# cindytsai/multigrid_poisson_solver

Hardware: AMD Instinct MI355X
Metric: vcycle_mlups (higher is better)
Workload: dtype f64; 1 GPU; V(3,3)-cycle N=8192^2 fp64, 11 levels to N=8, red-black GS(1e-7) coarse solve, cycle-file driver (eager, stream smoother: temporally blocked wave-streaming kernels on the large levels, register-tile kernels on the levels 65..1024, one-workgroup LDS kernel below; halos recomputed, neighbours via DPP lane shifts); N=8192, levels=11

## Files before the change

multigrid_poisson_solver_amd/csrc/mg_stream_impl.h:

```cpp
#include <hip/hip_runtime.h>

#include <type_traits>
#include <utility>

#include <algorithm>
#include <cstdlib>
#include <vector>

#include "mg_divconst.h"
#include "mg_internal.h"
#include "mg_lane_ops.h"

#if !defined(MG_REAL) || !defined(MG_REAL_NS)
#error "define MG_REAL (double|float) and MG_REAL_NS (f64|f32) before including mg_stream_impl.h"
#endif

namespace mg {
namespace k {
namespace MG_REAL_NS {

typedef MG_REAL real_t;

constexpr int PF_DEFAULT = 2;
#ifndef MG_WAVES_PER_WG
#define MG_WAVES_PER_WG 4
#endif
constexpr int WAVES_PER_WG = MG_WAVES_PER_WG;
constexpr int MAX_S = 4;
#ifndef MG_PF
#define MG_PF 2
#endif

constexpr bool recompute_instantiated(int pre, int steps)
{
    return MG_PF == 2 && pre >= 1 && steps >= 1 && pre <= MAX_S && steps <= MAX_S && pre + steps <= 6;
}

enum InMode { IN_LOAD = 0, IN_ZERO = 1, IN_PROLONG = 2 };

typedef real_t real2_t __attribute__((ext_vector_type(2)));
typedef real_t real4_t __attribute__((ext_vector_type(4)));

struct StreamParams {
    int N;
    real_t dx2, inv;
    const real_t *in;
    const real_t *F;
    real_t *out;
    real_t *D;
    int d_sign;
    double *part;
    long long *trace;
    int cols4;
    int rows_per_chunk;
    int groups;
    int n_blocks;
    int row_base, rows_local, own_y0, own_y1;
    int norm_y0, norm_y1;
    double *out_wide;
    int coarse_base, coarse_rows;
    int raw_norm;
    int nt_min_n;
    int no_out;
    int pre;
    int fc_base, fc_rows;
    const real_t *coarse;
    int Nc;
    const int *p_orow, *p_ocol;
    const real_t *p_rhi, *p_rlo, *p_chi, *p_clo;
    real_t c_dx, c_dx_rcp;
    real_t *Fc;
    int M;
    const int *r_inv;
    const real_t *r_w;
    const real_t *r_wf;
    const NodeBatchItem *batch;
    int part_stride;
    int n_batch;
    double *const *err_outs;
    real_t cw;
    int wt;
    real_t dc;
    int sh;
};


typedef const int __attribute__((address_space(4))) *const_int_ptr;
typedef const real_t __attribute__((address_space(4))) *const_real_ptr;
__device__ __forceinline__ int table_i(const int *t, int i) { return ((const_int_ptr)(uintptr_t)t)[i]; }
__device__ __forceinline__ real_t table_d(const real_t *t, int i) { return ((const_real_ptr)(uintptr_t)t)[i]; }

template <int COLS>
struct Row {
    real_t v[COLS];
};

#ifndef MG_ZERO_LEVEL1
#define MG_ZERO_LEVEL1 1
#endif
#ifndef MG_NT_LOADS
#define MG_NT_LOADS 0
#endif
template <int COLS, bool NT = false>
__device__ __forceinline__ Row<COLS> load_row(const real_t *__restrict__ row, unsigned col_bytes)
{
    Row<COLS> r;
    const char *a = reinterpret_cast<const char *>(row) + col_bytes;
    if constexpr (COLS == 2) {
        const real2_t t = NT ? __builtin_nontemporal_load(reinterpret_cast<const real2_t *>(a)) : *reinterpret_cast<const real2_t *>(a);
        r.v[0] = t.x;
        r.v[1] = t.y;
    } else if constexpr (COLS == 4) {
        const real4_t t = NT ? __builtin_nontemporal_load(reinterpret_cast<const real4_t *>(a)) : *reinterpret_cast<const real4_t *>(a);
        r.v[0] = t.x;
        r.v[1] = t.y;
        r.v[2] = t.z;
        r.v[3] = t.w;
    } else {
        r.v[0] = *reinterpret_cast<const real_t *>(a);
    }
    return r;
}

template <int COLS, bool NT>
__device__ __forceinline__ void store_row(real_t *__restrict__ row, unsigned col_bytes, const Row<COLS> &r)
{
    char *a = reinterpret_cast<char *>(row) + col_bytes;
    if constexpr (COLS == 2) {
        real2_t t;
        t.x = r.v[0];
        t.y = r.v[1];
        if constexpr (NT) __builtin_nontemporal_store(t, reinterpret_cast<real2_t *>(a));
        else *reinterpret_cast<real2_t *>(a) = t;
    } else if constexpr (COLS == 4) {
        real4_t t;
        t.x = r.v[0];
        t.y = r.v[1];
        t.z = r.v[2];
        t.w = r.v[3];
        if constexpr (NT) __builtin_nontemporal_store(t, reinterpret_cast<real4_t *>(a));
        else *reinterpret_cast<real4_t *>(a) = t;
    } else {
        *reinterpret_cast<real_t *>(a) = r.v[0];
    }
}

template <int S, bool RESTRICT, int COLS = 2>
struct Halo {
    static constexpr int A = COLS > 2 ? COLS : 2;
    static constexpr int value = (S + (RESTRICT ? 2 : 1) + A - 1) / A * A;
};


template <int NCV>
struct CoarseV {
    real_t v[NCV];
};
template <int NCV>
__device__ __forceinline__ CoarseV<NCV> load_coarse(const real_t *__restrict__ coarse, int Nc, int base, int rows, int row,
                                                    const unsigned (&col)[NCV])
{
    CoarseV<NCV> c;
    int r = row - base;
    r = r < 0 ? 0 : (r < rows - 1 ? r : rows - 1);
    const char *b = reinterpret_cast<const char *>(coarse + (size_t)r * Nc);
#pragma unroll
    for (int q = 0; q < NCV; ++q) c.v[q] = *reinterpret_cast<const real_t *>(b + col[q]);
    return c;
}


template <int NCV>
__device__ __forceinline__ CoarseV<NCV> load_coarse_local(const real_t *__restrict__ coarse, int Nc, int local_row, const unsigned (&col)[NCV])
{
    CoarseV<NCV> c;
    const char *b = reinterpret_cast<const char *>(coarse + (size_t)local_row * Nc);
#pragma unroll
    for (int q = 0; q < NCV; ++q) c.v[q] = *reinterpret_cast<const real_t *>(b + col[q]);
    return c;
}

template <class F, int... K>
__device__ __forceinline__ void unrolled_while(F &&f, std::integer_sequence<int, K...>)
{
    (void)(f(std::integral_constant<int, K>{}) && ...);
}

#ifndef MG_WPE_DOWN
#define MG_WPE_DOWN 0
#endif
template <int S, int COLS, int IN, bool RESTRICT, int PRE>
struct WavesPerSimd {
    static constexpr int min = (MG_WPE_DOWN > 0 && sizeof(real_t) == 8 && COLS == 2 && IN == 1  && RESTRICT && S <= 3) ? MG_WPE_DOWN : 1;
};

#ifndef MG_LDS_RING
#define MG_LDS_RING 1
#endif
#ifndef MG_PACKED_F32
#define MG_PACKED_F32 1
#endif
typedef float pk_t __attribute__((ext_vector_type(2)));
__device__ __forceinline__ pk_t pk(float a, float b)
{
    pk_t r;
    r.x = a;
    r.y = b;
    return r;
}
__device__ __forceinline__ pk_t pk_fma(pk_t a, pk_t b, pk_t c) { return __builtin_elementwise_fma(a, b, c); }
__device__ __forceinline__ pk_t pk_div_by_const(pk_t x, float c, float rc)
{
    const pk_t cc = pk(c, c), rr = pk(rc, rc);
    pk_t q = x * rr;
    pk_t r = pk_fma(-q, cc, x);
    q = pk_fma(r, rr, q);
    r = pk_fma(-q, cc, x);
    return pk_fma(r, rr, q);
}
template <int COLS, int PRE>
struct LdsRing {
    static constexpr bool value = MG_LDS_RING && PRE > 0 && (COLS == 2 || (COLS == 4 && sizeof(real_t) == 4));
};
template <int COLS> struct RingVec { typedef real_t full; typedef real_t half; };
template <> struct RingVec<2> { typedef real2_t full; typedef real_t half; };
template <> struct RingVec<4> { typedef real4_t full; typedef real2_t half; };
template <int COLS>
__device__ __forceinline__ typename RingVec<COLS>::full ring_pack(const Row<COLS> &r)
{
    typename RingVec<COLS>::full t;
    if constexpr (COLS == 1) t = r.v[0];
    else {
#pragma unroll
        for (int j = 0; j < COLS; ++j) t[j] = r.v[j];
    }
    return t;
}
template <int COLS>
__device__ __forceinline__ Row<COLS> ring_unpack(const typename RingVec<COLS>::full &t)
{
    Row<COLS> r;
    if constexpr (COLS == 1) r.v[0] = t;
    else {
#pragma unroll
        for (int j = 0; j < COLS; ++j) r.v[j] = t[j];
    }
    return r;
}
#ifndef MG_PF_UP
#define MG_PF_UP 3
#endif
#ifndef MG_PF_DOWN
#define MG_PF_DOWN 3
#endif
#ifndef MG_WPE_UP
#define MG_WPE_UP 2
#endif

template <bool SH>
__device__ __forceinline__ real_t minus_centre(real_t a, real_t u, real_t dc)
{
    if constexpr (SH) return a - dc * u;
    else return minus4(a, u);
}

template <int S, int COLS, int IN, bool RESTRICT, int PF = PF_DEFAULT, bool NT = false, int PRE = 0, bool WT = false, bool SH = false>
__global__ __launch_bounds__(64 * WAVES_PER_WG) __attribute__((amdgpu_waves_per_eu(LdsRing<COLS, PRE>::value ? MG_WPE_UP : WavesPerSimd<S, COLS, IN, RESTRICT, PRE>::min)))
void k_jacobi_stream(const StreamParams p)
{
    static_assert(COLS == 2 || COLS == 4 || (IN != IN_PROLONG && !RESTRICT), "fused transfer stages need column pairs");
    static_assert(COLS != 4 || sizeof(real_t) == 4, "4 columns per lane = one 16-byte access: fp32 fields only");
    constexpr int NCV = COLS / 2 + 2;
    constexpr int NS = COLS >= 2 ? COLS / 2 : 1;
    static_assert(PRE == 0 || (IN == IN_PROLONG && !RESTRICT), "recomputed pre-smoothing belongs to the fused `1` node");
    static_assert(!WT || (PRE == 0 && sizeof(real_t) == 8), "the weighted sweep: fp64 nodes that store and re-read U");
    static_assert(!SH || WT, "the screened operator is a form of the weighted sweep");
    constexpr int L = S + PRE;
    constexpr bool LDSR = LdsRing<COLS, PRE>::value;
    constexpr bool HALF = LDSR;
    constexpr bool PACKED = MG_PACKED_F32 && (COLS == 2 || COLS == 4) && sizeof(real_t) == 4;
#ifndef MG_TB_DIRECT
#define MG_TB_DIRECT 0
#endif
    constexpr bool TB_DIRECT = LDSR && MG_TB_DIRECT;
    constexpr int NB = LDSR ? 8 : (PF + L + 2 <= 8 ? 8 : 16);
    constexpr int NFR = LDSR ? (PF < 4 ? 4 : 8) : NB;
    static_assert((LDSR ? L + 2 <= NB : PF + L + 2 <= NB) && PF < 8, "the F ring has NB slots, the U ring 4 or 8");
    static_assert(!LDSR || (IN == IN_PROLONG && !RESTRICT), "the LDS ring belongs to the recomputing `1` node");
    typedef typename RingVec<COLS>::full ring_t;
    typedef typename RingVec<COLS>::half ringh_t;
    __shared__ ring_t s_g[LDSR ? WAVES_PER_WG : 1][LDSR ? NB : 1][LDSR ? 64 : 1];
    __shared__ ringh_t s_f[LDSR ? WAVES_PER_WG : 1][LDSR ? NB : 1][LDSR ? 64 : 1];
    constexpr int W = 64 * COLS;
    constexpr int H = Halo<L, RESTRICT, COLS>::value;
    constexpr int OW = W - 2 * H;

#ifdef MG_STREAM_TRACE
    const long long tr0 = wall_clock64();
#endif
    const int per_xcd = (p.n_blocks + 7) >> 3;
    const int tile = (int)(blockIdx.x & 7) * per_xcd + (int)(blockIdx.x >> 3);
    if (tile >= p.n_blocks) return;
    const real_t *a_in = p.in, *a_F = p.F, *a_coarse = p.coarse;
    real_t *a_out = p.out, *a_Fc = p.Fc;
    double *a_part = p.part;
    if (p.batch) {
        typedef const NodeBatchItem __attribute__((address_space(4))) *item_ptr;
        const item_ptr b = (item_ptr)(uintptr_t)(p.batch + blockIdx.y);
        a_in = static_cast<const real_t *>(b->in);
        a_F = static_cast<const real_t *>(b->F);
        a_coarse = static_cast<const real_t *>(b->coarse);
        a_out = static_cast<real_t *>(b->out);
        a_Fc = static_cast<real_t *>(b->Fc);
        if (a_part) a_part += (size_t)blockIdx.y * (size_t)p.part_stride;
    }
    const int chunk = tile / p.groups;
    const int group = tile - chunk * p.groups;

    const int lane = threadIdx.x & 63;
    const int wave = threadIdx.x >> 6;
    const int strip = group * WAVES_PER_WG + wave;
    const int N = p.N;
    const int own_x0 = strip * OW;
    if (own_x0 >= N) {
        if (a_part && lane == 0) a_part[(size_t)tile * WAVES_PER_WG + wave] = 0.0;
        return;
    }
    const int y0 = p.own_y0 + chunk * p.rows_per_chunk;
    int y1 = y0 + p.rows_per_chunk;
    if (y1 > p.own_y1) y1 = p.own_y1;
    if (y0 >= p.own_y1) return;
    const int av_lo = p.row_base > 0 ? p.row_base : 0;
    const int av_hi = p.row_base + p.rows_local < N ? p.row_base + p.rows_local : N;

    const int xl = own_x0 - H + lane * COLS;
    bool col_in[COLS], col_edge[COLS];
    bool lane_owns = true;
    real_t qc[COLS];
#pragma unroll
    for (int j = 0; j < COLS; ++j) {
        const int x = xl + j;
        col_in[j] = x >= 0 && x < N;
        col_edge[j] = x <= 0 || x >= N - 1;
        lane_owns = lane_owns && x >= own_x0 && x < own_x0 + OW && x < N;
        qc[j] = col_edge[j] ? real_t(0.0) : (WT ? p.cw : real_t(0.25));
    }
    int nm_even[COLS], nm_odd[COLS];
#pragma unroll
    for (int j = 0; j < COLS; ++j) {
        const bool mine = lane_owns && !col_edge[j];
        nm_even[j] = (mine && ((xl + j) & 1) == 0) ? -1 : 0;
        nm_odd[j] = (mine && ((xl + j) & 1) != 0) ? -1 : 0;
    }
    const bool lane_loads = col_in[0] && col_in[COLS - 1];
    const real_t dx2 = p.dx2, inv = p.inv;
    const real_t dc = SH ? p.dc : real_t(4.0);
    const bool want_res = RESTRICT || p.D != nullptr || p.part != nullptr;
    const unsigned col_off = (unsigned)(xl < 0 ? 0 : (xl > N - COLS ? N - COLS : xl)) * (unsigned)sizeof(real_t);
    const unsigned col_st = (unsigned)(xl < 0 ? 0 : xl) * (unsigned)sizeof(real_t);
    const unsigned row_bytes = (unsigned)N * (unsigned)sizeof(real_t);

    unsigned pc_col[NCV];
    int pc_cell[COLS];
    real_t pc_hi[COLS], pc_lo[COLS];
    real_t hA[COLS], hB[COLS];
#pragma unroll
    for (int q = 0; q < NCV; ++q) pc_col[q] = 0u;
#pragma unroll
    for (int j = 0; j < COLS; ++j) {
        pc_cell[j] = 0;
        pc_hi[j] = pc_lo[j] = hA[j] = hB[j] = real_t(0.0);
    }
    int c_row = -0x40000000;
    if constexpr (IN == IN_PROLONG) {
        if (lane_loads) {
            const int pc_base = p.p_ocol[xl];
            const int last = p.Nc - 1;
#pragma unroll
            for (int j = 0; j < COLS; ++j) {
                pc_cell[j] = p.p_ocol[xl + j] - pc_base;
                pc_hi[j] = p.p_chi[xl + j];
                pc_lo[j] = p.p_clo[xl + j];
            }
#pragma unroll
            for (int q = 0; q < NCV; ++q) pc_col[q] = (unsigned)(pc_base + q < last ? pc_base + q : last) * (unsigned)sizeof(real_t);
        }
    }
    auto interpolate = [&](const CoarseV<NCV> &c, real_t (&h)[COLS]) {
#pragma unroll
        for (int j = 0; j < COLS; ++j) {
            real_t ca = c.v[0], cb = c.v[1];
#pragma unroll
            for (int q = 1; q + 1 < NCV; ++q) {
                const bool here = pc_cell[j] == q;
                ca = here ? c.v[q] : ca;
                cb = here ? c.v[q + 1] : cb;
            }
            h[j] = ca * pc_hi[j] + cb * pc_lo[j];
        }
    };

    int rc_col[NS];
    bool rc_shift[NS];
    real_t rw_a[NS], rw_b[NS];
    Row<COLS> d_prev;
#pragma unroll
    for (int j = 0; j < COLS; ++j) d_prev.v[j] = 0.0;
#pragma unroll
    for (int q = 0; q < NS; ++q) {
        rc_col[q] = -1;
        rc_shift[q] = false;
        rw_a[q] = rw_b[q] = real_t(0.0);
    }
    if constexpr (RESTRICT) {
        if (lane_owns) {
#pragma unroll
            for (int q = 0; q < NS; ++q) {
                const int ca = p.r_inv[xl + 2 * q], cb = p.r_inv[xl + 2 * q + 1];
                rc_col[q] = ca >= 0 ? ca : cb;
                rc_shift[q] = ca < 0 && cb >= 0;
                if (rc_col[q] >= 0) {
                    rw_a[q] = p.r_w[rc_col[q]];
                    rw_b[q] = real_t(1.0) - rw_a[q];
                }
            }
        }
    }
    const bool first_col_lane = RESTRICT && lane_owns && xl == 0;
    const bool last_col_lane = RESTRICT && lane_owns && xl + COLS == N;
    if constexpr (RESTRICT) {
        for (int edge = 0; edge < 2; ++edge) {
            if (edge == 0 ? (y0 != 0) : (y1 != N)) continue;
            real_t *row = a_Fc + (size_t)((edge == 0 ? 0 : p.M - 1) - p.fc_base) * p.M;
#pragma unroll
            for (int q = 0; q < NS; ++q)
                if (rc_col[q] >= 0) row[rc_col[q]] = 0.0;
            if (first_col_lane) row[0] = 0.0;
            if (last_col_lane) row[p.M - 1] = 0.0;
        }
    }
    real_t ms[COLS];
#pragma unroll
    for (int j = 0; j < COLS; ++j) ms[j] = col_edge[j] ? real_t(0.0) : (p.d_sign < 0 ? real_t(-1.0) : real_t(1.0));

    constexpr bool EVEN_START = COLS >= 2;
    const int y0e = EVEN_START ? (y0 & ~1) : y0;
    const int y_first = y0e - (L + 1);
    const int T = (y1 - y0e) + 2 * (L + 1) + (RESTRICT ? 1 : 0);
    const int y_end = y_first + T;

    int tb_own = -1, tbn_own = -1;
    real_t tb_yh = 0.0, tb_yl = 0.0, tbn_yh = 0.0, tbn_yl = 0.0;
    int tb_rc = -1, tbn_rc = -1;
    real_t tb_rw = 0.0, tbn_rw = 0.0;
    auto load_own_block = [&](int first_row) {
        const int y = first_row + lane;
        const bool ok = y >= av_lo && y < av_hi && y < y_end;
        const int yc = y < 0 ? 0 : (y < N ? y : N - 1);
        const int v = p.p_orow[yc];
        tbn_own = ok ? v : -1;
    };
    auto load_weight_block = [&](int first_row) {
        const int y = first_row + lane;
        const int yc = y < 0 ? 0 : (y < N ? y : N - 1);
        tbn_yh = p.p_rhi[yc];
        tbn_yl = p.p_rlo[yc];
    };
    auto load_restrict_block = [&](int first_row) {
        const int y = first_row + lane;
        const bool ok = y >= y0 && y < y1;
        const int yc = y < 0 ? 0 : (y < N ? y : N - 1);
        const int v = p.r_inv[yc];
        const real_t w = p.r_wf[yc];
        tbn_rc = ok ? v : -1;
        tbn_rw = w;
    };
    const int yp_first = y_first - PRE;
    if constexpr (IN == IN_PROLONG) {
        load_own_block(yp_first);
        tb_own = tbn_own;
        load_weight_block(yp_first);
        tb_yh = tbn_yh;
        tb_yl = tbn_yl;
    }
    if constexpr (RESTRICT) {
        load_restrict_block(y_first - (L + 2));
        tb_rc = tbn_rc;
        tb_rw = tbn_rw;
    }

    Row<COLS> older[L + 1], newer[L + 1];
#pragma unroll
    for (int l = 0; l <= L; ++l)
#pragma unroll
        for (int j = 0; j < COLS; ++j) older[l].v[j] = newer[l].v[j] = 0.0;
    constexpr int NU = PF < 4 ? 4 : 8;
    Row<COLS> fr[NFR], pu[NU];
    CoarseV<NCV> pc[NU];
    int q_own[NU];
#pragma unroll
    for (int k = 0; k < NFR; ++k)
#pragma unroll
        for (int j = 0; j < COLS; ++j) fr[k].v[j] = 0.0;
#pragma unroll
    for (int k = 0; k < NU; ++k) {
#pragma unroll
        for (int j = 0; j < COLS; ++j) pu[k].v[j] = 0.0;
#pragma unroll
        for (int q = 0; q < NCV; ++q) pc[k].v[q] = 0.0;
        q_own[k] = -1;
    }

    if constexpr (LDSR) {
#pragma unroll
        for (int k = 0; k < NB; ++k) {
            s_g[wave][k][lane] = ring_t(real_t(0.0));
            s_f[wave][k][lane] = ringh_t(real_t(0.0));
        }
    }

    const char *in_b = reinterpret_cast<const char *>(a_in), *f_b = reinterpret_cast<const char *>(a_F);
    const int yc_first = y_first < av_lo ? av_lo : (y_first < av_hi ? y_first : av_hi - 1);
    unsigned long long ld_off = (unsigned long long)(yc_first - p.row_base) * row_bytes;
    int ld_t = 0;
    long long st_off = (long long)(y_first - L - p.row_base) * (long long)row_bytes;
    const unsigned inner_rows = (unsigned)(av_hi - av_lo - 1);

    auto fetch = [&](int u8) {
        if constexpr (IN != IN_ZERO && PRE == 0) pu[u8 % NU] = load_row<COLS, (MG_NT_LOADS >= 2)>(reinterpret_cast<const real_t *>(in_b + ld_off), col_off);
        fr[u8 % NFR] = load_row<COLS, (MG_NT_LOADS >= 1)>(reinterpret_cast<const real_t *>(f_b + ld_off), col_off);
        if constexpr (IN == IN_PROLONG) {
            const int own_s = lane_value(tb_own, ld_t & 63);
            q_own[u8 % NU] = own_s;
            const int cr = own_s + 1 - p.coarse_base;
            const int crc = cr < 0 ? 0 : (cr < p.coarse_rows - 1 ? cr : p.coarse_rows - 1);
            pc[u8 % NU] = load_coarse_local<NCV>(a_coarse, p.Nc, crc, pc_col);
        }
        ++ld_t;
        ld_off += ((unsigned)(y_first + ld_t - av_lo - 1) < inner_rows) ? row_bytes : 0u;
    };
#pragma unroll
    for (int k = 0; k < PF; ++k) fetch(k);

    if constexpr (IN == IN_PROLONG) {
        const int ys = yp_first > av_lo ? yp_first : av_lo;
        if (ys < av_hi && ys < y_end) {
            const int i0 = table_i(p.p_orow, ys);
            const CoarseV<NCV> c0 = load_coarse<NCV>(a_coarse, p.Nc, p.coarse_base, p.coarse_rows, i0, pc_col);
            interpolate(c0, hB);
            c_row = i0 - 1;
        }
    }

#ifdef MG_STREAM_TRACE
    const long long tr1 = wall_clock64();
#endif
    Row<COLS> gq[L + 1];
#pragma unroll
    for (int l = 0; l <= L; ++l)
#pragma unroll
        for (int j = 0; j < COLS; ++j) gq[l].v[j] = 0.0;
    double acc = 0.0;
    const unsigned rows_own = (unsigned)(y1 - y0), rows_norm = (unsigned)(p.norm_y1 - p.norm_y0);
    int nm_k0[COLS], nm_k1[COLS];
    const bool first_odd = ((y_first - L - 1) & 1) != 0;
    {
#pragma unroll
        for (int j = 0; j < COLS; ++j) {
            nm_k0[j] = first_odd ? nm_odd[j] : nm_even[j];
            nm_k1[j] = first_odd ? nm_even[j] : nm_odd[j];
        }
    }

    for (int t0 = 0; t0 < T; t0 += NB) {
        if ((t0 & 63) == 64 - NB) {
            if constexpr (IN == IN_PROLONG && !TB_DIRECT) {
                load_own_block(yp_first + t0 + NB);
                load_weight_block(yp_first + t0 + NB);
            }
            if constexpr (RESTRICT) load_restrict_block(y_first + t0 + NB - (L + 2));
        }
        if ((t0 & 63) == 0 && t0 > 0) {
            if constexpr (IN == IN_PROLONG && TB_DIRECT) {
                load_weight_block(yp_first + t0);
            }
            if constexpr (IN == IN_PROLONG) {
                tb_yh = tbn_yh;
                tb_yl = tbn_yl;
            }
            if constexpr (RESTRICT) {
                tb_rc = tbn_rc;
                tb_rw = tbn_rw;
            }
        }
        auto row_step = [&](auto k_tag) -> bool {
            constexpr int k = decltype(k_tag)::value;
            const int t = t0 + k;
            if (!LDSR && k > 0 && t >= T) return false;
            const int yin = y_first + t;
            Row<COLS> nw;
            if constexpr (IN == IN_ZERO || PRE > 0) {
#pragma unroll
                for (int j = 0; j < COLS; ++j) nw.v[j] = 0.0;
            } else {
                nw = pu[k % NU];
            }
            const int own_i = q_own[k % NU];
            if constexpr (IN == IN_PROLONG) {
                if (k == NB - PF && (t0 & 63) == 64 - NB) {
                    if constexpr (TB_DIRECT) load_own_block(yp_first + t0 + NB);
                    tb_own = tbn_own;
                }
                if (own_i >= 0 && own_i != c_row) {
                    asm volatile("" ::);
#pragma unroll
                    for (int j = 0; j < COLS; ++j) hA[j] = hB[j];
                    c_row = own_i;
                    interpolate(pc[k % NU], hB);
                }
            }
            fetch((k + PF) % NB);

            auto add_prolongation = [&](Row<COLS> &row) {
                if (own_i >= 0) {
                    const real_t own_yh = lane_value(tb_yh, t & 63), own_yl = lane_value(tb_yl, t & 63);
                    const real_t c_dx = p.c_dx, c_rcp = p.c_dx_rcp;
                    if constexpr (PACKED) {
#pragma unroll
                        for (int j = 0; j < COLS; j += 2) {
                            const pk_t yh2 = pk((float)own_yh, (float)own_yh), yl2 = pk((float)own_yl, (float)own_yl);
                            const pk_t num = pk((float)hA[j], (float)hA[j + 1]) * yh2 + pk((float)hB[j], (float)hB[j + 1]) * yl2;
                            const pk_t pv = pk_div_by_const(pk_div_by_const(num, (float)c_dx, (float)c_rcp), (float)c_dx, (float)c_rcp);
                            const pk_t sum = pk((float)row.v[j], (float)row.v[j + 1]) + pv;
                            row.v[j] = sum.x;
                            row.v[j + 1] = sum.y;
                        }
                    } else {
#pragma unroll
                        for (int j = 0; j < COLS; ++j) {
                            const real_t num = hA[j] * own_yh + hB[j] * own_yl;
                            const real_t pv = div_by_const(div_by_const(num, c_dx, c_rcp), c_dx, c_rcp);
                            row.v[j] = row.v[j] + pv;
                        }
                    }
                }
            };
            if constexpr (IN == IN_PROLONG && PRE == 0) add_prolongation(nw);

#pragma unroll
            for (int l = 1; l <= L; ++l) {
                const int y = yin - l;
                const int inner = ((unsigned)(y - 1) < (unsigned)(N - 2)) ? -1 : 0;
                const Row<COLS> c = newer[l - 1], so = older[l - 1];
                Row<COLS> g;
                if constexpr (LDSR) {
                    g = gq[l];
                } else {
                    const Row<COLS> &f = fr[(k - l + NB) % NB];
#pragma unroll
                    for (int j = 0; j < COLS; ++j) g.v[j] = dx2 * f.v[j];
                }
                const real_t west0 = from_lane_below(c.v[COLS - 1]);
                const real_t east_last = from_lane_above(c.v[0]);
                Row<COLS> o;
                if constexpr (PACKED) {
#pragma unroll
                    for (int P = 0; P < COLS / 2; ++P) {
                        const int a = 2 * P, b = 2 * P + 1;
                        const pk_t q2 = pk((float)hi_bits_and(qc[a], inner), (float)hi_bits_and(qc[b], inner));
                        const pk_t g2 = pk((float)g.v[a], (float)g.v[b]);
                        pk_t o2;
                        if ((IN == IN_ZERO || PRE > 0) && MG_ZERO_LEVEL1 && l == 1) {
                            o2 = pk_fma(q2, -g2, pk(0.0f, 0.0f));
                        } else {
                            const pk_t c2 = pk((float)c.v[a], (float)c.v[b]);
                            const pk_t e2 = pk((float)c.v[b], (float)(b == COLS - 1 ? east_last : c.v[b < COLS - 1 ? b + 1 : 0]));
                            const pk_t w2 = pk((float)(a == 0 ? west0 : c.v[a > 0 ? a - 1 : 0]), (float)c.v[a]);
                            pk_t t2 = pk((float)nw.v[a], (float)nw.v[b]) + pk((float)so.v[a], (float)so.v[b]);
                            t2 = t2 + e2;
                            t2 = t2 + w2;
                            t2 = pk_fma(pk(-4.0f, -4.0f), c2, t2) - g2;
                            o2 = pk_fma(q2, t2, c2);
                        }
                        o.v[a] = o2.x;
                        o.v[b] = o2.y;
                    }
                    older[l - 1] = c;
                    newer[l - 1] = nw;
                    nw = o;
                    if constexpr (IN == IN_PROLONG && PRE > 0) {
                        if (l == PRE) add_prolongation(nw);
                    }
                    continue;
                }
                if constexpr ((IN == IN_ZERO || PRE > 0) && MG_ZERO_LEVEL1) {
                    if (l == 1) {
#pragma unroll
                        for (int j = 0; j < COLS; ++j) {
                            if constexpr (WT) o.v[j] = fused_mul_add(inner ? qc[j] : real_t(0.0), -g.v[j], real_t(0.0));
                            else o.v[j] = fused_mul_add(hi_bits_and(qc[j], inner), -g.v[j], real_t(0.0));
                        }
                        older[l - 1] = c;
                        newer[l - 1] = nw;
                        nw = o;
                        if constexpr (IN == IN_PROLONG && PRE > 0) {
                            if (l == PRE) add_prolongation(nw);
                        }
                        continue;
                    }
                }
#pragma unroll
                for (int j = 0; j < COLS; ++j) {
                    const real_t w = j == 0 ? west0 : c.v[j > 0 ? j - 1 : 0];
                    const real_t e = j == COLS - 1 ? east_last : c.v[j < COLS - 1 ? j + 1 : 0];
                    const real_t t4 = minus_centre<SH>(nw.v[j] + so.v[j] + e + w, c.v[j], dc) - g.v[j];
                    if constexpr (WT) o.v[j] = c.v[j] + (inner ? qc[j] : real_t(0.0)) * t4;
                    else o.v[j] = fused_mul_add(hi_bits_and(qc[j], inner), t4, c.v[j]);
                }
                older[l - 1] = c;
                newer[l - 1] = nw;
                nw = o;
                if constexpr (IN == IN_PROLONG && PRE > 0) {
                    if (l == PRE) add_prolongation(nw);
                }
            }

            if constexpr (LDSR) {
                const Row<COLS> &fin = fr[k % NFR];
                Row<COLS> gin;
#pragma unroll
                for (int j = 0; j < COLS; ++j) gin.v[j] = dx2 * fin.v[j];
                s_g[wave][k % NB][lane] = ring_pack<COLS>(gin);
                constexpr int par = (k + L + 1) & 1;
                if constexpr (COLS == 2) {
                    s_f[wave][k % NB][lane] = fin.v[par];
                } else {
                    ringh_t h;
                    h.x = fin.v[par];
                    h.y = fin.v[par + 2];
                    s_f[wave][k % NB][lane] = h;
                }
#pragma unroll
                for (int l = 1; l <= L; ++l) {
                    gq[l] = ring_unpack<COLS>(s_g[wave][(k + 1 - l + 2 * NB) % NB][lane]);
                }
            }

            {
                const int y = yin - L;
                if ((unsigned)(y - y0) < rows_own && lane_owns && !p.no_out) {
                    if (sizeof(real_t) != sizeof(double) && p.out_wide) {
                        double *w = reinterpret_cast<double *>(reinterpret_cast<char *>(p.out_wide) + 2 * st_off + 2u * col_st);
                        typedef double wide2_t __attribute__((ext_vector_type(2)));
                        if constexpr (COLS % 2 == 0) {
#pragma unroll
                            for (int j = 0; j < COLS; j += 2) {
                                wide2_t t;
                                t.x = (double)nw.v[j];
                                t.y = (double)nw.v[j + 1];
                                if (COLS == 2) __builtin_nontemporal_store(t, reinterpret_cast<wide2_t *>(w + j));
                                else *reinterpret_cast<wide2_t *>(w + j) = t;
                            }
                        } else {
#pragma unroll
                            for (int j = 0; j < COLS; ++j) __builtin_nontemporal_store((double)nw.v[j], w + j);
                        }
                    } else {
                        store_row<COLS, NT>(reinterpret_cast<real_t *>(reinterpret_cast<char *>(a_out) + st_off), col_st, nw);
                    }
                }
            }

            if (want_res) {
                const int y = yin - L - 1;
                const bool mine_row = (unsigned)(y - y0) < rows_own;
                const int inner = ((unsigned)(y - 1) < (unsigned)(N - 2)) ? -1 : 0;
                const int cm = (mine_row && (unsigned)(y - p.norm_y0) < rows_norm) ? inner : 0;
                const Row<COLS> c = newer[L], so = older[L];
                if constexpr (HALF) {
                    const ringh_t fh = s_f[wave][(k - L - 1 + 2 * NB) % NB][lane];
#pragma unroll
                    for (int j = k & 1; j < COLS; j += 2) {
                        real_t fv;
                        if constexpr (COLS == 2) fv = fh;
                        else fv = fh[j >> 1];
                        const real_t w = j == 0 ? from_lane_below(c.v[COLS - 1]) : c.v[j > 0 ? j - 1 : 0];
                        const real_t e = j == COLS - 1 ? from_lane_above(c.v[0]) : c.v[j < COLS - 1 ? j + 1 : 0];
                        const real_t r = inv * minus4(nw.v[j] + so.v[j] + e + w, c.v[j]) - fv;
                        const int am = ((lane_owns && !col_edge[j]) ? -1 : 0) & cm;
                        acc += fabs(bits_and((double)r, am));
                    }
                    older[L] = newer[L];
                    newer[L] = nw;
                    st_off += row_bytes;
                    return true;
                }
                const Row<COLS> &f = fr[(k - L - 1 + 2 * NB) % NFR];
                const real_t west0 = from_lane_below(c.v[COLS - 1]);
                const real_t east_last = from_lane_above(c.v[0]);
                Row<COLS> d;
#pragma unroll
                for (int j = 0; j < COLS; ++j) {
                    const real_t w = j == 0 ? west0 : c.v[j > 0 ? j - 1 : 0];
                    const real_t e = j == COLS - 1 ? east_last : c.v[j < COLS - 1 ? j + 1 : 0];
                    const real_t r = inv * minus_centre<SH>(nw.v[j] + so.v[j] + e + w, c.v[j], dc) - f.v[j];
                    if constexpr (RESTRICT) {
                        d.v[j] = r * hi_bits_and(ms[j], inner);
                    } else {
                        d.v[j] = r;
                    }
                    if constexpr (EVEN_START) {
                        if ((j & 1) == (k & 1)) acc += fabs(bits_and((double)r, ((lane_owns && !col_edge[j]) ? -1 : 0) & cm));
                    } else {
                        const int am = ((k & 1) ? nm_k1[j] : nm_k0[j]) & cm;
                        acc += fabs(bits_and((double)r, am));
                    }
                }
                if constexpr (!RESTRICT) {
                    if (mine_row && lane_owns && p.D) {
                        Row<COLS> ds;
#pragma unroll
                        for (int j = 0; j < COLS; ++j) {
                            const real_t dv = (inner != 0 && !col_edge[j]) ? d.v[j] : real_t(0.0);
                            ds.v[j] = p.d_sign < 0 ? -dv : dv;
                        }
                        store_row<COLS, false>(reinterpret_cast<real_t *>(reinterpret_cast<char *>(p.D) + (st_off - (long long)row_bytes)), col_st, ds);
                    }
                } else {
                    if (mine_row && lane_owns && p.D)
                        store_row<COLS, false>(reinterpret_cast<real_t *>(reinterpret_cast<char *>(p.D) + (st_off - (long long)row_bytes)), col_st, d);
                }

                if constexpr (RESTRICT) {
                    const int rc_row = lane_value(tb_rc, t & 63);
                    if (rc_row >= 0) {
                        const real_t wc = lane_value(tb_rw, t & 63), wd = real_t(1.0) - wc;
                        const real_t p_up = from_lane_above(d_prev.v[0]);
                        const real_t q_up = from_lane_above(d.v[0]);
                        real_t *crow = a_Fc + (size_t)(rc_row - p.fc_base) * p.M;
#pragma unroll
                        for (int q = 0; q < NS; ++q) {
                            const real_t p_next = q + 1 < NS ? d_prev.v[q + 1 < NS ? 2 * q + 2 : 0] : p_up;
                            const real_t q_next = q + 1 < NS ? d.v[q + 1 < NS ? 2 * q + 2 : 0] : q_up;
                            const real_t u0 = rc_shift[q] ? d_prev.v[2 * q + 1] : d_prev.v[2 * q];
                            const real_t u1 = rc_shift[q] ? p_next : d_prev.v[2 * q + 1];
                            const real_t u2 = rc_shift[q] ? d.v[2 * q + 1] : d.v[2 * q];
                            const real_t u3 = rc_shift[q] ? q_next : d.v[2 * q + 1];
                            const real_t vc = rw_b[q] * wd * u0 + rw_a[q] * wd * u1 + wc * rw_b[q] * u2 + rw_a[q] * wc * u3;
                            if (rc_col[q] >= 0) crow[rc_col[q]] = vc;
                        }
                        if (first_col_lane) crow[0] = 0.0;
                        if (last_col_lane) crow[p.M - 1] = 0.0;
                    }
                    d_prev = d;
                }
            }
            older[L] = newer[L];
            newer[L] = nw;
            st_off += row_bytes;
            return true;
        };
        unrolled_while(row_step, std::make_integer_sequence<int, NB>{});
    }
#ifdef MG_STREAM_TRACE
    if (p.trace && (threadIdx.x & 63) == 0) {
        const long long tr2 = wall_clock64();
        long long *rec = p.trace + 8 + 4 * ((size_t)tile * WAVES_PER_WG + wave);
        rec[0] = tr0;
        rec[1] = tr1;
        rec[2] = tr2;
        rec[3] = (long long)blockIdx.x;
        if (tile == p.n_blocks / 2 && wave == 0) {
            p.trace[0] = tr0;
            p.trace[1] = tr1;
            p.trace[2] = tr2;
            p.trace[3] = T;
        }
    }
#endif
    if (a_part) {
#pragma unroll
        for (int o = 32; o > 0; o >>= 1) acc += __shfl_down(acc, o, 64);
        if (lane == 0) a_part[(size_t)tile * WAVES_PER_WG + wave] = acc;
    }
}

#ifndef MG_STREAM_KERNEL_ONLY
template <int S, int COLS, int IN, bool RESTRICT, int PF = PF_DEFAULT, bool NT = false, int PRE = 0, bool WT = false, bool SH = false>
void launch_k(hipStream_t s, StreamParams p, double *err_out)
{
    static int blocks_per_cu = 0;
    if (blocks_per_cu == 0) {
        int n = 0;
        if (hipOccupancyMaxActiveBlocksPerMultiprocessor(&n, k_jacobi_stream<S, COLS, IN, RESTRICT, PF, NT, PRE, WT, SH>, 64 * WAVES_PER_WG, 0) != hipSuccess || n < 1) {
            (void)hipGetLastError();
            n = 2;
        }
        blocks_per_cu = n > 8 ? 8 : n;
    }
    const int N = p.N;
    const int own = p.own_y1 - p.own_y0;
    if (own <= 0) return;
    constexpr int OW = 64 * COLS - 2 * Halo<S + PRE, RESTRICT, COLS>::value;
    const int strips = (N + OW - 1) / OW;
    const int groups = (strips + WAVES_PER_WG - 1) / WAVES_PER_WG;
    static const int resident_pct = [] { const char *e = getenv("MG_RESIDENT_PCT"); return e ? atoi(e) : 100; }();
    const int resident = ctx().n_cu * blocks_per_cu * resident_pct / 100;
    const int nb = p.batch ? p.n_batch : 1;
    int chunks = resident / (groups * nb);
    static const int min_rows_forced = [] { const char *e = getenv("MG_MIN_ROWS"); return e ? atoi(e) : 0; }();
    const int min_rows = min_rows_forced ? min_rows_forced : (N <= 256 ? 2 : N <= 1024 ? 4 : 8);
    const int max_chunks = (own + min_rows - 1) / min_rows;
    if (chunks > max_chunks) chunks = max_chunks;
    if (chunks < 1) chunks = 1;
    int rows = (own + chunks - 1) / chunks;
    static const int rows_cap = [] { const char *e = getenv("MG_MAX_ROWS"); return e ? atoi(e) : 0; }();
    if (rows_cap > 0 && rows > rows_cap) rows = rows_cap;
    if (LdsRing<COLS, PRE>::value) {
        const int march = rows + 2 * (S + PRE + 1);
        rows += (8 - march % 8) % 8;
    } else if (COLS >= 2) {
        rows += rows & 1;
    }
    chunks = (own + rows - 1) / rows;
    p.rows_per_chunk = rows;
    p.groups = groups;
    p.n_blocks = chunks * groups;
    if (ctx().geometry_log)
        stream_geometry_record({N, own, rows, chunks, groups, nb, S, COLS, IN, (int)RESTRICT, PRE,
                                (NT ? MG_GEOMETRY_NT : 0) | (WT ? MG_GEOMETRY_WT : 0) | (SH ? MG_GEOMETRY_SH : 0) |
                                    (sizeof(real_t) == 4 ? MG_GEOMETRY_F32 : 0)});
    p.part = nullptr;
#ifdef MG_STREAM_TRACE
    static long long *trace_dev = nullptr;
    if (!trace_dev) (void)hipMalloc((void **)&trace_dev, (8 + 4 * 4 * 4096) * sizeof(long long));
    (void)hipMemsetAsync(trace_dev, 0, (8 + 4 * 4 * 4096) * sizeof(long long), s);
    p.trace = trace_dev;
#endif
    const size_t n_part = (size_t)p.n_blocks * WAVES_PER_WG;
    const bool want_norm = err_out || (p.batch && p.err_outs);
    if (want_norm) {
        p.part = norm_partials(n_part * (size_t)nb);
        if (!p.part) return;
    }
    p.part_stride = (int)n_part;
    const int grid = ((p.n_blocks + 7) / 8) * 8;
    hipLaunchKernelGGL((k_jacobi_stream<S, COLS, IN, RESTRICT, PF, NT, PRE, WT, SH>), dim3(grid, nb), dim3(64 * WAVES_PER_WG), 0, s, p);
#ifdef MG_STREAM_TRACE
    {
        long long t[4];
        (void)hipStreamSynchronize(s);
        (void)hipMemcpy(t, trace_dev, sizeof t, hipMemcpyDeviceToHost);
        fprintf(stderr, "[stream trace] N=%d IN=%d R=%d tiles=%d rows/chunk=%d: prologue %.2f us, %lld steps %.2f us (%.3f us/step)\n", N, IN, (int)RESTRICT,
                p.n_blocks, rows, (t[1] - t[0]) * 0.01, t[3], (t[2] - t[1]) * 0.01, (t[2] - t[1]) * 0.01 / (double)t[3]);
        if (N >= 4096 && p.n_blocks <= 4096) {
            const size_t nw = (size_t)p.n_blocks * WAVES_PER_WG;
            std::vector<long long> all(4 * nw);
            (void)hipMemcpy(all.data(), trace_dev + 8, all.size() * sizeof(long long), hipMemcpyDeviceToHost);
            long long t_min = 0x7fffffffffffffffll, t_max = 0;
            std::vector<double> start, life, endt;
            for (size_t w = 0; w < nw; ++w) {
                if (all[4 * w] == 0) continue;
                if (all[4 * w] < t_min) t_min = all[4 * w];
                if (all[4 * w + 2] > t_max) t_max = all[4 * w + 2];
            }
            double xcd_end[8] = {0}, xcd_start[8] = {0};
            for (size_t w = 0; w < nw; ++w) {
                if (all[4 * w] == 0) continue;
                start.push_back((all[4 * w] - t_min) * 0.01);
                endt.push_back((all[4 * w + 2] - t_min) * 0.01);
                life.push_back((all[4 * w + 2] - all[4 * w]) * 0.01);
                const int x = (int)(all[4 * w + 3] & 7);
                if (endt.back() > xcd_end[x]) xcd_end[x] = endt.back();
                if (start.back() > xcd_start[x]) xcd_start[x] = start.back();
            }
            auto pct = [](std::vector<double> v, double q) { std::sort(v.begin(), v.end()); return v[(size_t)(q * (v.size() - 1))]; };
            fprintf(stderr, "   waves %zu: start p50 %.1f p99 %.1f max %.1f us | lifetime p1 %.1f p50 %.1f p99 %.1f max %.1f | end p1 %.1f p50 %.1f p99 %.1f max %.1f | span %.1f us\n",
                    nw, pct(start, .5), pct(start, .99), pct(start, 1.0), pct(life, .01), pct(life, .5), pct(life, .99), pct(life, 1.0), pct(endt, .01),
                    pct(endt, .5), pct(endt, .99), pct(endt, 1.0), (t_max - t_min) * 0.01);
            fprintf(stderr, "   last wave per XCD ends at:");
            for (int x = 0; x < 8; ++x) fprintf(stderr, " %.1f", xcd_end[x]);
            fprintf(stderr, " us\n");
        }
    }
#endif
    if (p.batch && p.err_outs) {
        for (int i = 0; i < nb; ++i)
            if (p.err_outs[i]) norm_finish(s, p.part + (size_t)i * n_part, n_part, p.raw_norm ? -1 : N, p.err_outs[i]);
    } else if (err_out) {
        norm_finish(s, p.part, n_part, p.raw_norm ? -1 : N, err_out);
    }
}

template <int S, int PF>
void launch_variant(hipStream_t s, const StreamParams &p, double *err_out)
{
    const bool restrict_out = p.Fc != nullptr, prolong_in = p.coarse != nullptr, zero = p.in == nullptr;
    const bool nt = p.N >= p.nt_min_n;
    if constexpr (sizeof(real_t) == 4) {
        if (p.cols4 && !(prolong_in && p.pre)) {
            if (restrict_out) {
                if (zero) launch_k<S, 4, IN_ZERO, true, PF>(s, p, err_out);
                else launch_k<S, 4, IN_LOAD, true, PF>(s, p, err_out);
            } else if (prolong_in) {
                if (nt) launch_k<S, 4, IN_PROLONG, false, PF, true>(s, p, err_out);
                else launch_k<S, 4, IN_PROLONG, false, PF>(s, p, err_out);
            } else {
                if (zero) launch_k<S, 4, IN_ZERO, false, PF>(s, p, err_out);
                else launch_k<S, 4, IN_LOAD, false, PF>(s, p, err_out);
            }
            return;
        }
    }
    if constexpr (sizeof(real_t) == 8) {
        if (p.wt) {
            auto weighted = [&](auto sh_tag) {
                constexpr bool SH = decltype(sh_tag)::value;
                if (p.N % 2 != 0) {
                    if (zero) launch_k<S, 1, IN_ZERO, false, PF, false, 0, true, SH>(s, p, err_out);
                    else launch_k<S, 1, IN_LOAD, false, PF, false, 0, true, SH>(s, p, err_out);
                } else if (restrict_out) {
                    if (zero) launch_k<S, 2, IN_ZERO, true, (PF == 2 && S <= 3 ? MG_PF_DOWN : PF), false, 0, true, SH>(s, p, err_out);
                    else launch_k<S, 2, IN_LOAD, true, PF, false, 0, true, SH>(s, p, err_out);
                } else if (prolong_in) {
                    if (p.pre != 0) fail(MG_ERR_UNSUPPORTED, "jacobi_stream: no recomputing `1` node for the weighted sweep");
                    else if (nt) launch_k<S, 2, IN_PROLONG, false, PF, true, 0, true, SH>(s, p, err_out);
                    else launch_k<S, 2, IN_PROLONG, false, PF, false, 0, true, SH>(s, p, err_out);
                } else {
                    if (zero) launch_k<S, 2, IN_ZERO, false, PF, false, 0, true, SH>(s, p, err_out);
                    else launch_k<S, 2, IN_LOAD, false, PF, false, 0, true, SH>(s, p, err_out);
                }
            };
            if (p.sh) weighted(std::true_type{});
            else weighted(std::false_type{});
            return;
        }
    }
    if (p.N % 2 != 0) {
        if (zero) launch_k<S, 1, IN_ZERO, false, PF>(s, p, err_out);
        else launch_k<S, 1, IN_LOAD, false, PF>(s, p, err_out);
    } else if (restrict_out) {
        if (zero) launch_k<S, 2, IN_ZERO, true, (PF == 2 && S <= 3 ? MG_PF_DOWN : PF)>(s, p, err_out);
        else launch_k<S, 2, IN_LOAD, true, PF>(s, p, err_out);
    } else if (prolong_in) {
        if (p.pre != 0) {
            bool done = false;
            auto with_pre = [&](auto pre_tag) {
                constexpr int PRE = decltype(pre_tag)::value;
                if constexpr (recompute_instantiated(PRE, S) && PF == 2) {
                    if (p.pre == PRE && !done) {
                        constexpr int PFU = LdsRing<2, PRE>::value ? MG_PF_UP : PF;
                        if (nt) launch_k<S, 2, IN_PROLONG, false, PFU, true, PRE>(s, p, err_out);
                        else launch_k<S, 2, IN_PROLONG, false, PFU, false, PRE>(s, p, err_out);
                        done = true;
                    }
                }
            };
            with_pre(std::integral_constant<int, 1>{});
            with_pre(std::integral_constant<int, 2>{});
            with_pre(std::integral_constant<int, 3>{});
            with_pre(std::integral_constant<int, 4>{});
            if (!done) fail(MG_ERR_UNSUPPORTED, "jacobi_stream: no recomputing `1` node for %d + %d sweeps, prefetch depth %d", p.pre, S, PF);
            return;
        }
        if (nt) launch_k<S, 2, IN_PROLONG, false, PF, true>(s, p, err_out);
        else launch_k<S, 2, IN_PROLONG, false, PF>(s, p, err_out);
    } else {
        if (zero) launch_k<S, 2, IN_ZERO, false, PF>(s, p, err_out);
        else launch_k<S, 2, IN_LOAD, false, PF>(s, p, err_out);
    }
}

template <int S>
void launch_steps(hipStream_t s, const StreamParams &p, double *err_out)
{
    if constexpr (S <= 3 && MG_PF == 3) launch_variant<S, 3>(s, p, err_out);
    else launch_variant<S, 2>(s, p, err_out);
}


inline void run(hipStream_t s, const SmoothNode<real_t> &nd)
{
    const int N = nd.N, steps = nd.steps, pre = nd.pre;
    const RowWindow *fine_w = nd.fine_w;
    if (nd.batch && (fine_w || nd.coarse_w || nd.fc_w || nd.D || nd.out_wide || nd.batch->n < 1)) {
        fail(MG_ERR_ARG, "jacobi_stream: a batch of instances runs whole grids without a stored residual");
        return;
    }
    if (pre != 0 && !(recompute_instantiated(pre, steps) && nd.coarse && !nd.Fc)) {
        fail(MG_ERR_ARG, "jacobi_stream: recomputed pre-smoothing exists for pre + steps <= 6 sweeps of the fused `1` node (pre=%d steps=%d)", pre, steps);
        return;
    }
    if ((nd.cw != 0.25 || nd.shifted) && (pre != 0 || sizeof(real_t) != 8)) {
        fail(MG_ERR_ARG, "jacobi_stream: the weighted sweep runs fp64 nodes that store and re-read U");
        return;
    }
    if (pre != 0 && nd.D) {
        fail(MG_ERR_ARG, "jacobi_stream: the recomputing `1` node forms the error norm only, it stores no residual");
        return;
    }
    if (steps < 1 || steps > MAX_S) {
        fail(MG_ERR_ARG, "jacobi_stream: %d sweeps per launch (1..%d)", steps, MAX_S);
        return;
    }
    if ((nd.coarse || nd.Fc) && (N < 4 || N % 2 != 0)) {
        fail(MG_ERR_ARG, "jacobi_stream: fused transfer stages need an even grid size (N=%d)", N);
        return;
    }
    StreamParams p = {};
    if (nd.batch) {
        p.batch = nd.batch->dev;
        p.n_batch = nd.batch->n;
        p.err_outs = nd.batch->err_outs;
    }
    p.N = N;
    p.dx2 = nd.dx2;
    p.inv = nd.inv;
    p.in = nd.in;
    p.F = nd.F;
    p.out = nd.out;
    p.out_wide = nd.out_wide;
    p.pre = pre;
    p.no_out = nd.no_out ? 1 : 0;
    p.cw = (real_t)nd.cw;
    p.wt = nd.cw != 0.25 ? 1 : 0;
    if (nd.shifted) {
        p.dc = (real_t)nd.dc;
        p.sh = p.wt = 1;
    }
    p.D = nd.D;
    p.d_sign = nd.d_sign;
    p.row_base = fine_w ? fine_w->base : 0;
    p.rows_local = fine_w ? fine_w->rows : N;
    p.own_y0 = fine_w ? fine_w->own_lo : 0;
    p.own_y1 = fine_w ? fine_w->own_hi : N;
    p.norm_y0 = fine_w && fine_w->norm_lo >= 0 ? fine_w->norm_lo : p.own_y0;
    p.norm_y1 = fine_w && fine_w->norm_lo >= 0 ? fine_w->norm_hi : p.own_y1;
    p.raw_norm = fine_w ? 1 : 0;
    static const int cols4_min = [] { const char *e = getenv("MG_F32_COLS4_MIN_N"); return e ? atoi(e) : 8192; }();
    p.cols4 = (sizeof(real_t) == 4 && N % 4 == 0 && N >= cols4_min && (!nd.coarse || nd.pt->fusable4)) ? 1 : 0;
    static const int nt_min = [] { const char *e = getenv("MG_NT_MIN_N"); return e ? atoi(e) : 8192; }();
    p.nt_min_n = nt_min;
    if (nd.coarse) {
        const ProlongTable &pt = *nd.pt;
        p.coarse_base = nd.coarse_w ? nd.coarse_w->base : 0;
        p.coarse_rows = nd.coarse_w ? nd.coarse_w->rows : nd.Nc;
        p.coarse = nd.coarse;
        p.Nc = nd.Nc;
        p.p_orow = pt.owner_row;
        p.p_ocol = pt.owner_col;
        p.p_rhi = weights_as(real_t(), pt.row_hi, pt.row_hi_f);
        p.p_rlo = weights_as(real_t(), pt.row_lo, pt.row_lo_f);
        p.p_chi = weights_as(real_t(), pt.col_hi, pt.col_hi_f);
        p.p_clo = weights_as(real_t(), pt.col_lo, pt.col_lo_f);
        p.c_dx = (real_t)pt.c_dx;
        p.c_dx_rcp = (real_t)1 / p.c_dx;
    }
    if (nd.Fc) {
        const RestrictTable &rt = *nd.rt;
        p.fc_base = nd.fc_w ? nd.fc_w->base : 0;
        p.fc_rows = nd.fc_w ? nd.fc_w->rows : nd.M;
        p.Fc = nd.Fc;
        p.M = nd.M;
        p.r_inv = rt.inv;
        p.r_w = weights_as(real_t(), rt.w, rt.w_f);
        p.r_wf = weights_as(real_t(), rt.inv_w, rt.inv_w_f);
    }
    switch (steps) {
        case 1: launch_steps<1>(s, p, nd.err); break;
        case 2: launch_steps<2>(s, p, nd.err); break;
        case 3: launch_steps<3>(s, p, nd.err); break;
        default: launch_steps<4>(s, p, nd.err); break;
    }
}

#endif

}
}
}
```

Measured before the change: 815,600 MLUPS.

## Skip smoother and residual work on seam fill rows of temporally blocked stream kernel

Splits the wave-streaming loop body into templated variants. The first one or two bodies become a fill phase that skips the stencil update for time levels whose rows are still inside the recomputed halo seam and simply rotate the register rows. A residual-guard variant restricts residual accumulation to owned rows. This removes redundant halo arithmetic in the pipeline fill at the cost of more code (larger instruction footprint) and a config-dependent exclusion list.

```diff
diff --git a/multigrid_poisson_solver_amd/csrc/mg_stream_impl.h b/multigrid_poisson_solver_amd/csrc/mg_stream_impl.h
--- a/multigrid_poisson_solver_amd/csrc/mg_stream_impl.h
+++ b/multigrid_poisson_solver_amd/csrc/mg_stream_impl.h
@@ -98,6 +98,9 @@
 #ifndef MG_ZERO_LEVEL1
 #define MG_ZERO_LEVEL1 1
 #endif
+#ifndef MG_SEAM_SKIP
+#define MG_SEAM_SKIP 1
+#endif
 #ifndef MG_NT_LOADS
 #define MG_NT_LOADS 0
 #endif
@@ -192,6 +195,12 @@
 template <int S, int COLS, int IN, bool RESTRICT, int PRE>
 struct WavesPerSimd {
     static constexpr int min = (MG_WPE_DOWN > 0 && sizeof(real_t) == 8 && COLS == 2 && IN == 1  && RESTRICT && S <= 3) ? MG_WPE_DOWN : 1;
+};
+template <int S, int COLS, int IN, bool RESTRICT, int PRE, bool WT>
+struct SeamSkip {
+    static constexpr bool kept_out = sizeof(real_t) == 8 && S == 4 && COLS == 2 && IN == 1  && !RESTRICT && WT;
+    static constexpr bool one_body = IN == 2  && PRE == 0;
+    static constexpr int form = (MG_SEAM_SKIP == 0 || kept_out) ? 0 : one_body ? 2 : 1;
 };
 
 #ifndef MG_LDS_RING
@@ -572,7 +581,9 @@
         }
     }
 
-    for (int t0 = 0; t0 < T; t0 += NB) {
+    const int fill = y0 - y0e;
+    auto run_body = [&](const int t0, auto guarded_tag) __attribute__((always_inline)) {
+        constexpr int GUARDED = decltype(guarded_tag)::value;
         if ((t0 & 63) == 64 - NB) {
             if constexpr (IN == IN_PROLONG && !TB_DIRECT) {
                 load_own_block(yp_first + t0 + NB);
@@ -649,6 +660,13 @@
 
 #pragma unroll
             for (int l = 1; l <= L; ++l) {
+                if constexpr (GUARDED == 1) {
+                    if (t < fill + 2 * l) {
+                        older[l - 1] = newer[l - 1];
+                        newer[l - 1] = nw;
+                        continue;
+                    }
+                }
                 const int y = yin - l;
                 const int inner = ((unsigned)(y - 1) < (unsigned)(N - 2)) ? -1 : 0;
                 const Row<COLS> c = newer[l - 1], so = older[l - 1];
@@ -771,7 +789,9 @@
                 }
             }
 
-            if (want_res) {
+            bool res_live = want_res;
+            if constexpr (GUARDED != 0) res_live = want_res && (unsigned)(yin - L - 1 - y0) < rows_own + (RESTRICT ? 1u : 0u);
+            if (res_live) {
                 const int y = yin - L - 1;
                 const bool mine_row = (unsigned)(y - y0) < rows_own;
                 const int inner = ((unsigned)(y - 1) < (unsigned)(N - 2)) ? -1 : 0;
@@ -861,6 +881,23 @@
             return true;
         };
         unrolled_while(row_step, std::make_integer_sequence<int, NB>{});
+    };
+    typedef std::integral_constant<int, 0> plain_body;
+    typedef std::integral_constant<int, 1> fill_body;
+    typedef std::integral_constant<int, 2> residual_guard_body;
+    int t_steady = 0;
+    constexpr int SEAM = SeamSkip<S, COLS, IN, RESTRICT, PRE, WT>::form;
+    if constexpr (SEAM == 1) {
+        constexpr int FILL_BODIES = (2 * (L + 1) + NB - 1) / NB;
+        static_assert(FILL_BODIES <= 2, "the fill of a pipeline of L <= 7 levels ends in the second body");
+        run_body(0, fill_body{});
+        if constexpr (FILL_BODIES == 2) run_body(NB, fill_body{});
+        t_steady = FILL_BODIES * NB;
+    }
+    if constexpr (SEAM == 2) {
+        for (int t0 = 0; t0 < T; t0 += NB) run_body(t0, residual_guard_body{});
+    } else {
+        for (int t0 = t_steady; t0 < T; t0 += NB) run_body(t0, plain_body{});
     }
 #ifdef MG_STREAM_TRACE
     if (p.trace && (threadIdx.x & 63) == 0) {
```

Measured after the change: 827,000 MLUPS, median of 3. About the same (+1.4%).
